# deveshv-99/mlir-HashJoin

Measured on AMD Instinct MI355X. Metric: probed tuples/sec + joined rows/sec, |R|=|S|=2^28 int64 keys, higher is better.
Workload: dtype int64

## Files before the change

### mlir-hashjoin_amd/csrc/hj_capi.cpp

```cpp
#include <hip/hip_runtime.h>

#include <cstdio>
#include <cstdlib>
#include <atomic>
#include <cmath>
#include <cstring>
#include <map>
#include <mutex>
#include <string>
#include <functional>
#include <thread>
#include <type_traits>
#include <vector>

#include "hj.h"
#include "hj_internal.h"

using hj::kNarrow;
using hj::kWide;

namespace {

thread_local std::string g_err;

// ... 384 lines not shown
}

hj::BucketSet bucket_set(SetBufs &sb) {
    hj::BucketSet b;
    b.rows = sb.rows.p;
    b.bbin = (unsigned *)sb.bbin.p;
    b.bfill = (unsigned *)sb.bfill.p;
    b.runs = (unsigned long long *)sb.runs.p;
    b.rstart = (unsigned long long *)sb.rstart.p;
    b.max_buckets = sb.max_buckets;
    b.max_rows = sb.max_rows;
    b.max_runs = sb.max_runs;
    return b;
}

int ensure_radix_scratch(hj_ctx *c, SetBufs &fin, int64_t n, bool wide, const hj::RadixPlan &pl, int routed_src = 0) {
    const size_t P = size_t(1) << pl.total_bits, esz = wide ? 16 : 8;
    HJ_TRY(ensure_set(fin, hj::radix_need(n, pl, true, routed_src), esz, P, hj::kFinalPbl));
    if (pl.passes > 1) HJ_TRY(ensure_set(c->tset, hj::radix_need(n, pl, false, routed_src), esz, P, hj::kPassPbl));
    HJ_TRY(ensure_buf(c->nb, 16));
    HJ_TRY(ensure_buf(c->pcur, (P + 1) * 8));
    HJ_TRY(ensure_buf(c->rcur, (P + 1) * 8));
    HJ_TRY(ensure_buf(c->tile_start, (P + 1) * 4));
    HJ_TRY(ensure_buf(c->tile_owner, (size_t)hj::radix_tiles(n, (int)P) * 4));
    HJ_TRY(ensure_buf(c->tdesc, (size_t)hj::radix_tiles(n, (int)P) * 16));
    HJ_TRY(ensure_buf(c->wstart, 1025 * 4));
    const size_t items = (size_t)hj::radix_join_items(pl, fin.max_runs);
    HJ_TRY(ensure_buf(c->work_start, (size_t)hj::radix_work_words(pl, fin.max_runs) * 4));
    HJ_TRY(ensure_buf(c->work_desc, items * hj::radix_item_desc_bytes()));
    HJ_TRY(ensure_buf(c->scan_sums, ((P + 1) / 8192 + 2) * 8));
    HJ_TRY(ensure_buf(c->raw_cnt, 2 * hj::kRawCntWords * 8));
    {
        const size_t had = c->scan_state.bytes;
        HJ_TRY(ensure_buf(c->scan_state, ((P + 1) / 1024 + 4) * 8));
        if (c->scan_state.bytes != had) HJ_HIP(hipMemset(c->scan_state.p, 0, c->scan_state.bytes));
    }
    return HJ_OK;
}

hj::RadixWork radix_work(hj_ctx *c) {
    hj::RadixWork w;
    w.tmp = bucket_set(c->tset);
    w.nb = (unsigned *)c->nb.p;
    w.pcur = (unsigned long long *)c->pcur.p;
    w.rcur = (unsigned long long *)c->rcur.p;
    w.tile_start = (unsigned *)c->tile_start.p;
    w.tile_owner = (unsigned *)c->tile_owner.p;
    w.tdesc = c->tdesc.p;
    w.wstart = (unsigned *)c->wstart.p;
    w.scan_sums = (unsigned long long *)c->scan_sums.p;
    w.scan_state = (unsigned long long *)c->scan_state.p;
    w.raw_cnt = (unsigned long long *)c->raw_cnt.p;
    w.work_start = (unsigned *)c->work_start.p;
    w.work_desc = c->work_desc.p;
    return w;
}

int choose_strategy(const hj_ctx *c, int64_t n_build) {
    if (c->strategy == HJ_STRATEGY_GLOBAL || c->strategy == HJ_STRATEGY_RADIX) return c->strategy;
    if (n_build >= kRadixMinRows) return HJ_STRATEGY_RADIX;
    if (n_build >= kDualMinBuildRows && c->probe_hint >= radix_probe_min_rows(n_build)) return HJ_STRATEGY_RADIX;
    return HJ_STRATEGY_GLOBAL;
}

struct RadixSrc {
    hj::SrcDev src;
    const uint64_t *counts = nullptr;
// ... 1837 lines not shown
```

### mlir-hashjoin_amd/csrc/hj_radix.hip

```cpp
#include <cstdint>
#include <cstdlib>
#include <type_traits>

#include "hj.h"
#include "hj_internal.h"

namespace hj {
namespace {

typedef unsigned long long u64;
constexpr int kTile = 4096;
constexpr int kPassThreads = 1024;
constexpr int kPassRows = kTile / kPassThreads;
constexpr int kMaxFan = 512;
constexpr int kSmallPassThreads = 512;
constexpr int kSmallFan = 256;
constexpr int kJoinItems = 5;
constexpr int kJoinSub = 8;
constexpr int kPackedRow = 3;
constexpr int kBucketed = 4;
constexpr unsigned kNoBucket = 0xFFFFFFFFu;

__device__ __forceinline__ u64 rhash(u64 k) { return radix_hash(k); }

// ... 111 lines not shown
__global__ __launch_bounds__(1024) void k_scan_blocks(u64 *a, u64 n, u64 *sums) {
    __shared__ u64 wsum[16];
    const u64 base = (u64)blockIdx.x * kScanBlock + (u64)threadIdx.x * kScanPer;
    u64 v[kScanPer], s = 0;
#pragma unroll
    for (int i = 0; i < kScanPer; ++i) {
        v[i] = (base + i < n) ? a[base + i] : 0ull;
        s += v[i];
    }
    u64 total;
    u64 run = block_excl_scan<1024>(s, wsum, &total);
#pragma unroll
    for (int i = 0; i < kScanPer; ++i) {
        if (base + i < n) a[base + i] = run;
        run += v[i];
    }
    if (threadIdx.x == 0) sums[blockIdx.x] = total;
}

__global__ __launch_bounds__(1024) void k_scan_add(u64 *a, u64 n, const u64 *sums) {
    __shared__ u64 wsum[16];
    if (blockIdx.x == 0) return;
    u64 v = 0;
    for (unsigned i = threadIdx.x; i < blockIdx.x; i += 1024) v += sums[i];
    u64 add;
    block_excl_scan<1024>(v, wsum, &add);
    const u64 base = (u64)blockIdx.x * kScanBlock;
    for (int i = threadIdx.x; i < kScanBlock; i += 1024)
        if (base + i < n) a[base + i] += add;
}

__device__ __forceinline__ unsigned runs_of(unsigned fill) { return (fill + (1u << kRunLog) - 1) >> kRunLog; }

constexpr u64 kLbAgg = 1ull << 62, kLbInc = 2ull << 62, kLbVal = (1ull << 62) - 1;
constexpr int kLbThreads = 256, kLbPer = 4, kLbTile = kLbThreads * kLbPer;

struct ChunkMapArgs {
    const u64 *off_a, *off_b;
    unsigned chunk;
    bool split;
    unsigned *start, *owner;
};

template <bool MAP>
__global__ __launch_bounds__(kLbThreads) void k_scan_lb(u64 *a, u64 n, u64 *state, ChunkMapArgs mp) {
    __shared__ u64 wsum[16];
    __shared__ u64 s_pre;
    __shared__ unsigned s_tile;
    const unsigned nt = (unsigned)((n + kLbTile - 1) / kLbTile);
    if (threadIdx.x == 0) s_tile = (unsigned)atomicAdd(&state[nt], 1ull);
    __syncthreads();
    const unsigned t = s_tile;
    const u64 base = (u64)t * kLbTile + (u64)threadIdx.x * kLbPer;
    u64 v[kLbPer], s = 0;
#pragma unroll
    for (int i = 0; i < kLbPer; ++i) {
        const u64 e = base + i;
        if constexpr (MAP) {
            v[i] = 0ull;
            if (e + 1 < n) {
                const u64 len = mp.off_a[e + 1] - mp.off_a[e];
                const bool live = mp.off_b ? (mp.off_b[e + 1] > mp.off_b[e]) : true;
                const u64 c = live ? (len + mp.chunk - 1) / mp.chunk : 0ull;
                v[i] = mp.split && c >= 2 ? c | (c << 31) : c;
            }
        } else {
            v[i] = e < n ? a[e] : 0ull;
        }
        s += v[i];
    }
    u64 total;
    u64 run = block_excl_scan<kLbThreads>(s, wsum, &total);
    if (threadIdx.x < 64) {
        const unsigned lane = threadIdx.x;
        u64 pre = 0;
        if (t == 0) {
            if (lane == 0) atomicExch(&state[0], kLbInc | total);
        } else {
            if (lane == 0) atomicExch(&state[t], kLbAgg | total);
            for (unsigned w = t; w > 0;) {
                const u64 x = lane < w ? atomicOr(&state[w - 1 - lane], 0ull) : kLbInc;
                const u64 inc = __ballot((x >> 62) == 2ull), none = __ballot((x >> 62) == 0ull);
                const u64 upto = inc ? (inc & (~inc + 1ull)) * 2ull - 1ull : ~0ull;
                if (none & upto) {
                    __builtin_amdgcn_s_sleep(1);
                    continue;
                }
                pre += wave_incl_add64((upto >> lane) & 1ull && lane < w ? (x & kLbVal) : 0ull);
                pre = __shfl(pre, 63);
                if (inc) break;
                w = w > 64u ? w - 64u : 0u;
            }
            if (lane == 0) atomicExch(&state[t], kLbInc | (pre + total));
        }
        if (lane == 0) s_pre = pre;
    }
    __syncthreads();
    run += s_pre;
#pragma unroll
    for (int i = 0; i < kLbPer; ++i) {
        const u64 e = base + i;
        if (e < n) {
            if constexpr (MAP) {
                const unsigned lo = (unsigned)(run & 0x7FFFFFFFull);
                a[e] = ((run >> 31) << 32) | lo;
                mp.start[e] = lo;
                const unsigned c = (unsigned)(v[i] & 0x7FFFFFFFull);
                for (unsigned k = 0; k < c; ++k) mp.owner[lo + k] = (unsigned)e;
            } else {
                a[e] = run;
            }
        }
        run += v[i];
    }
    __syncthreads();
    if (threadIdx.x == 0) {
        __threadfence();
        if (atomicAdd(&state[nt + 1], 1ull) == (u64)nt - 1ull) {
            __threadfence();
            for (unsigned k = 0; k < nt + 2; ++k) atomicExch(&state[k], 0ull);
        }
    }
}

struct PassArgs {
    SrcDev in;
    u64 n;
    bool cols_aligned;
    const void *in_rows;
    const u64 *in_runs;
    const u64 *in_rstart;
    u64 in_max_rows, in_max_runs;
    const unsigned *tile_start;
    const struct TileDesc *tdesc;
    int nseg;
    void *out_rows;
    unsigned *bbin, *bfill, *nb;
    const unsigned *wstart;
    unsigned max_buckets;
    int out_pbl;
    int shift;
    int fbits;
    u64 *prof = nullptr;
    u64 *rcnt = nullptr;
    const u64 *slot_base = nullptr;
    u64 out_max_rows = 0;
    int hash_top = 0;
    unsigned tile_rows = kTile;
};

struct TileDesc {
    u64 lo;
    unsigned cnt, seg;
};

// ... 463 lines not shown
        zero_a[i] = 0ull;
        zero_b[i] = 0ull;
    }
    if (blockIdx.x != 0) return;
    const unsigned w = threadIdx.x;
    const unsigned T_ = bucketed ? a.tile_start[a.nseg] : (unsigned)((a.n + a.tile_rows - 1) / a.tile_rows);
    u64 q = 0;
    if (w < G) {
        const unsigned t0 = (unsigned)((u64)w * T_ / G), t1 = (unsigned)((u64)(w + 1) * T_ / G);
        if (t1 > t0) {
            const u64 segs = bucketed ? (u64)(a.tdesc[t1 - 1].seg - a.tdesc[t0].seg + 1) : 1ull;
            const u64 PB = 1ull << a.out_pbl;
            q = ((u64)(t1 - t0) * a.tile_rows + PB - 1) / PB + segs * (1ull << a.fbits) + 1;
        }
    }
    u64 tot;
    const u64 pre = block_excl_scan<1024>(q, wsum, &tot);
    if (w <= G) wstart[w] = (unsigned)(pre < a.max_buckets ? pre : a.max_buckets);
    if (w == G) *a.nb = (unsigned)(tot < a.max_buckets ? tot : a.max_buckets);
}

constexpr int kPlanSegs = 4096;
struct TilePlanArgs {
    PassArgs a;
    const u64 *rstart;
    unsigned G, tb;
    unsigned *tile_start;
    TileDesc *desc;
    unsigned *wstart;
    u64 *zero_a, *zero_b;
    u64 zero_n;
};

__device__ __forceinline__ void tile_plan_body(const TilePlanArgs &p, unsigned bid, unsigned nblk) {
    const PassArgs &a = p.a;
    const u64 *rstart = p.rstart;
    const unsigned G = p.G, tb = p.tb;
    unsigned *tile_start = p.tile_start;
    TileDesc *desc = p.desc;
    unsigned *wstart = p.wstart;
    u64 *zero_a = p.zero_a, *zero_b = p.zero_b;
    const u64 zero_n = p.zero_n;
    __shared__ unsigned ts[kPlanSegs + 1];
    __shared__ u64 wsum[16];
    constexpr int PER = kPlanSegs / 1024;
    const int nseg = a.nseg;
    const unsigned rpt = a.tile_rows >> kRunLog;
    unsigned c[PER], sum = 0;
#pragma unroll
    for (int i = 0; i < PER; ++i) {
        const int sg = threadIdx.x * PER + i;
        c[i] = sg < nseg ? (unsigned)((rstart[sg + 1] - rstart[sg] + rpt - 1) / rpt) : 0u;
        sum += c[i];
    }
    u64 total;
    u64 run = block_excl_scan<1024>(sum, wsum, &total);
#pragma unroll
    for (int i = 0; i < PER; ++i) {
        const int sg = threadIdx.x * PER + i;
        if (sg < nseg) ts[sg] = (unsigned)run;
        run += c[i];
    }
    if (threadIdx.x == 0) ts[nseg] = (unsigned)total;
    __syncthreads();
    const unsigned T = (unsigned)total;
    auto seg_of_tile = [&](unsigned t) -> unsigned {
        unsigned lo = 0, hi = (unsigned)nseg;
        while (hi - lo > 1) {
            const unsigned mid = (lo + hi) >> 1;
            if (ts[mid] <= t) lo = mid;
            else hi = mid;
        }
        return lo;
    };
    for (unsigned t = bid * 1024 + threadIdx.x; t < T && t < tb; t += nblk * 1024) {
        const unsigned sg = seg_of_tile(t);
        const u64 lo = rstart[sg] + (u64)(t - ts[sg]) * rpt;
        const u64 e = rstart[sg + 1];
        TileDesc d;
        d.lo = lo;
        d.cnt = (unsigned)(e - lo < (u64)rpt ? e - lo : (u64)rpt);
        d.seg = sg;
        desc[t] = d;
    }
    for (u64 i = (u64)bid * 1024 + threadIdx.x; i < zero_n; i += (u64)nblk * 1024) {
        zero_a[i] = 0ull;
        zero_b[i] = 0ull;
    }
    if (bid != 0) return;
    for (int sg = threadIdx.x; sg <= nseg; sg += 1024) tile_start[sg] = ts[sg];
    const unsigned w = threadIdx.x;
    u64 q = 0;
    if (w < G) {
        const unsigned t0 = (unsigned)((u64)w * T / G), t1 = (unsigned)((u64)(w + 1) * T / G);
        if (t1 > t0) {
            const u64 segs = (u64)(seg_of_tile(t1 - 1) - seg_of_tile(t0) + 1);
            const u64 PB = 1ull << a.out_pbl;
            q = ((u64)(t1 - t0) * a.tile_rows + PB - 1) / PB + segs * (1ull << a.fbits) + 1;
        }
    }
    u64 tot;
    const u64 pre = block_excl_scan<1024>(q, wsum, &tot);
    if (w <= G) wstart[w] = (unsigned)(pre < a.max_buckets ? pre : a.max_buckets);
    if (w == G) *a.nb = (unsigned)(tot < a.max_buckets ? tot : a.max_buckets);
}

__global__ __launch_bounds__(1024) void k_tile_plan(TilePlanArgs p) { tile_plan_body(p, blockIdx.x, gridDim.x); }

constexpr int kListPer = 4;
constexpr int kListLds = 4096;


struct PlaceArgs {
    const unsigned *bbin, *bfill, *nb;
    unsigned max_buckets;
    int pbl;
    const u64 *rstart;
    u64 *rcur, *runs;
    int P;
    const u64 *raw = nullptr;
};
static_assert(kRawCntWords == (u64)kPlanSegs + 1, "raw count words: a plan's segments + 1");

__device__ __forceinline__ void bplace_body(const PlaceArgs &pa, unsigned bid) {
    const unsigned *bbin = pa.bbin, *bfill = pa.bfill, *nb = pa.nb;
    const unsigned max_buckets = pa.max_buckets;
    const int pbl = pa.pbl;
    const u64 *rstart = pa.rstart;
    u64 *rcur = pa.rcur, *runs = pa.runs;
    const int P = pa.P;
    __shared__ unsigned cr[kListLds];
    __shared__ u64 cbr[kListLds];
    const unsigned n = *nb < max_buckets ? *nb : max_buckets;
    const u64 base = (u64)bid * 1024 * kListPer;
    if (base >= n) return;
    const unsigned lane_ = threadIdx.x & 63u;
    auto put_runs = [&](bool ok, u64 j, unsigned f, u64 at) {
        const int rl = pbl > kRunLog ? (pbl - kRunLog < 6 ? pbl - kRunLog : 6) : 0;
        const unsigned R = 1u << rl, k0 = lane_ & (R - 1u);
        for (unsigned b0 = 0; b0 < 64u; b0 += 64u >> rl) {
            const int src = (int)(b0 + (lane_ >> rl));
            const bool o = __shfl((int)ok, src) != 0;
            const unsigned fs = (unsigned)__shfl((int)f, src);
            const u64 js = ((u64)(unsigned)__shfl((int)(j >> 32), src) << 32) | (unsigned)__shfl((int)j, src);
            const u64 as = ((u64)(unsigned)__shfl((int)(at >> 32), src) << 32) | (unsigned)__shfl((int)at, src);
            for (unsigned k = k0; o && (k << kRunLog) < fs; k += R) {
                const unsigned cnt = fs - (k << kRunLog) < (1u << kRunLog) ? fs - (k << kRunLog) : (1u << kRunLog);
                runs[as + k] = ((((u64)js << pbl) + ((u64)k << kRunLog)) << 7) | cnt;
            }
        }
    };
    if (P > kListLds) {
        const unsigned lane = threadIdx.x & 63u;
        unsigned bi[kListPer], fi[kListPer], pre[kListPer], l0i[kListPer];
        u64 ri[kListPer];
#pragma unroll
        for (int i = 0; i < kListPer; ++i) {
            const u64 j = base + (u64)i * 1024 + threadIdx.x;
            bi[i] = j < n ? bbin[j] : kNoBucket;
            const bool valid = bi[i] < (unsigned)P;
            fi[i] = valid ? bfill[j] : 0u;
            const unsigned nr = runs_of(fi[i]);
            const u64 vm = __ballot(valid);
            l0i[i] = vm ? (unsigned)__ffsll((long long)vm) - 1u : 64u;
            ri[i] = 0ull;
            pre[i] = 0u;
            if (!vm) continue;
            const unsigned b0 = (unsigned)__builtin_amdgcn_readlane((int)bi[i], (int)l0i[i]);
            const bool same = valid && bi[i] == b0;
            const unsigned v = same ? nr : 0u;
            const unsigned incl = wave_incl_add(v);
            const unsigned tot = (unsigned)__builtin_amdgcn_readlane((int)incl, 63);
            pre[i] = same ? incl - v : ~0u;
            if (valid && !same) ri[i] = atomicAdd(&rcur[bi[i]], (u64)nr);
            if (lane == l0i[i]) ri[i] = atomicAdd(&rcur[b0], (u64)tot);
        }
#pragma unroll
        for (int i = 0; i < kListPer; ++i) {
            if (l0i[i] == 64u) continue;
            const unsigned b0 = (unsigned)__builtin_amdgcn_readlane((int)bi[i], (int)l0i[i]);
            const u64 g = ((u64)(unsigned)__builtin_amdgcn_readlane((int)(ri[i] >> 32), (int)l0i[i]) << 32) |
                          (u64)(unsigned)__builtin_amdgcn_readlane((int)ri[i], (int)l0i[i]);
            const bool ok = bi[i] < (unsigned)P;
            const u64 j = base + (u64)i * 1024 + threadIdx.x;
            const u64 at = !ok ? 0ull : (pre[i] != ~0u ? rstart[b0] + g + pre[i] : rstart[bi[i]] + ri[i]);
            put_runs(ok, j, fi[i], at);
        }
        return;
    }
    for (int i = threadIdx.x; i < P; i += 1024) cr[i] = 0u;
    __syncthreads();
    unsigned rr[kListPer], bn[kListPer], fl[kListPer];
#pragma unroll
    for (int i = 0; i < kListPer; ++i) {
        const u64 j = base + (u64)i * 1024 + threadIdx.x;
        bn[i] = j < n ? bbin[j] : kNoBucket;
        if (bn[i] >= (unsigned)P) bn[i] = kNoBucket;
        fl[i] = bn[i] != kNoBucket ? bfill[j] : 0u;
        if (bn[i] != kNoBucket) rr[i] = atomicAdd(&cr[bn[i]], runs_of(fl[i]));
    }
    __syncthreads();
    for (int i = threadIdx.x; i < P; i += 1024)
        if (cr[i]) cbr[i] = rstart[i] + atomicAdd(&rcur[i], (u64)cr[i]);
    __syncthreads();
#pragma unroll
    for (int i = 0; i < kListPer; ++i) {
        const u64 j = base + (u64)i * 1024 + threadIdx.x;
        const bool ok = bn[i] != kNoBucket;
        put_runs(ok, j, fl[i], ok ? cbr[bn[i]] + rr[i] : 0ull);
    }
}

__global__ __launch_bounds__(1024) void k_bplace(PlaceArgs pa) { bplace_body(pa, blockIdx.x); }

__global__ __launch_bounds__(1024) void k_place_plan(PlaceArgs pa, unsigned nplace, TilePlanArgs tp) {
    __shared__ u64 rs[kPlanSegs + 1];
    if (pa.raw) {
        __shared__ u64 wsum[16];
        constexpr int PER = (kPlanSegs + 1 + 1023) / 1024;
        const int n = pa.P + 1;
        u64 v[PER], sum = 0;
#pragma unroll
        for (int i = 0; i < PER; ++i) {
            const int e = threadIdx.x * PER + i;
            v[i] = e < n ? pa.raw[e] : 0ull;
            sum += v[i];
        }
        u64 total;
        u64 run = block_excl_scan<1024>(sum, wsum, &total);
#pragma unroll
        for (int i = 0; i < PER; ++i) {
            const int e = threadIdx.x * PER + i;
            if (e < n) {
                rs[e] = run;
                if (blockIdx.x == 0) ((u64 *)pa.rstart)[e] = run;
            }
            run += v[i];
        }
        __syncthreads();
        pa.rstart = rs;
        tp.rstart = rs;
    }
    if (blockIdx.x < nplace) bplace_body(pa, blockIdx.x);
    else tile_plan_body(tp, blockIdx.x - nplace, gridDim.x - nplace);
}

struct JoinArgs {
    const void *r, *s;
    const u64 *r_runs, *s_runs;
    const u64 *r_rstart, *s_rstart;
    int P;
    const unsigned *work_start;
    const struct ItemDesc *desc;
    int tshift;
    void *out_r, *out_s;
    long long cap;
    u64 *counter;
    u64 *dup_flag;
    unsigned *defer = nullptr, *defer_n = nullptr;
    const unsigned *list = nullptr, *list_n = nullptr;
    const u64 *sample = nullptr;
    unsigned modes = 7u;
    unsigned *next_item = nullptr;
    bool empty_s = false;
    bool all_if_mode2 = false;
    const u64 *skip_if_set = nullptr;
};

constexpr unsigned kModeUnique = 1u, kModeSome = 2u, kModeMostlyRepeated = 4u;
constexpr unsigned kModesAll = kModeUnique | kModeSome | kModeMostlyRepeated;
constexpr int kSampleParts = 64;

typedef __attribute__((address_space(4))) const u64 cu64_t;
__device__ __forceinline__ u64 sload(const u64 *p) { return *(cu64_t *)p; }

__host__ __device__ __forceinline__ int sample_mode(u64 rows, u64 repeats) {
    return repeats * 4 > rows ? 2 : (repeats * 64 >= rows && repeats ? 1 : 0);
// ... 2429 lines not shown
        a.in = src;
        a.n = n;
        a.cols_aligned = ((((uintptr_t)src.key) | ((uintptr_t)src.pay)) & 15) == 0;
        a.in_rows = prev ? prev->rows : nullptr;
        a.in_runs = prev ? prev->runs : nullptr;
        a.in_rstart = prev ? prev->rstart : nullptr;
        a.in_max_rows = prev ? prev->max_rows : 0;
        a.in_max_runs = prev ? prev->max_runs : 0;
        a.tile_start = ws.tile_start;
        a.tdesc = nullptr;
        a.nseg = nseg;
        a.out_rows = dst.rows;
        a.bbin = dst.bbin;
        a.bfill = dst.bfill;
        a.nb = nbw;
        {
            const u64 by_rows = dst.max_rows >> pl.pbl[pass];
            a.max_buckets = (unsigned)(by_rows < dst.max_buckets ? by_rows : dst.max_buckets);
        }
        a.out_pbl = pl.pbl[pass];
        a.shift = shift;
        a.fbits = fb;
        a.tile_rows = pass_tile_rows(fb, wide);
        a.wstart = ws.wstart;
        const u64 P = (u64)nseg << fb;
        const bool fuse = ws.raw_cnt && pass + 1 < pl.passes && P <= (u64)kPlanSegs;
        u64 *cnt = fuse ? ws.raw_cnt + (u64)(pass & 1) * kRawCntWords : dst.rstart;
        a.rcnt = n > 0 ? cnt : nullptr;
        if (grid > 1023) return hipErrorInvalidValue;
        const unsigned zgrid = blocks_for(P + 1, 1024);
        if (prev && nseg <= kPlanSegs) {
            const u64 tb = radix_tiles((long long)n, nseg);
            a.tdesc = (const TileDesc *)ws.tdesc;
            unsigned pg = blocks_for(tb, 1024);
            if (pg < zgrid) pg = zgrid;
            if (pg > 1024) pg = 1024;
            TilePlanArgs tp{a, (const u64 *)prev->rstart, grid, (unsigned)tb, ws.tile_start, (TileDesc *)ws.tdesc,
                            ws.wstart, cnt, rcur, P + 1};
            if (pending) hipLaunchKernelGGL(k_place_plan, dim3(np_prev + pg), dim3(1024), 0, st, pa_prev, np_prev, tp);
            else hipLaunchKernelGGL(k_tile_plan, dim3(pg), dim3(1024), 0, st, tp);
            pending = false;
        } else {
            place_alone();
            if (prev) {
                const unsigned rpt = a.tile_rows >> kRunLog;
                chunk_map(prev->rstart, nullptr, nseg, rpt, ws.tile_start, ws.tile_owner, ws.pcur, ws.scan_sums, st,
                          (u64)n / (u64)(nseg > 0 ? nseg : 1) / (u64)a.tile_rows);
                const u64 tb = radix_tiles((long long)n, nseg);
                hipLaunchKernelGGL(k_tile_desc, dim3(blocks_for(tb, 256)), dim3(256), 0, st,
                                   (const unsigned *)ws.tile_start, (const unsigned *)ws.tile_owner,
                                   (const u64 *)prev->rstart, nseg, (unsigned)tb, (TileDesc *)ws.tdesc, rpt);
                a.tdesc = (const TileDesc *)ws.tdesc;
            }
            hipLaunchKernelGGL(k_id_plan, dim3(zgrid < 1024 ? zgrid : 1024), dim3(1024), 0, st, a, prev != nullptr, grid,
                               ws.wstart, cnt, rcur, P + 1);
        }
        if (n > 0) {
#define HJ_PASS(W, FORM)                                                                                    \
    do {                                                                                                    \
        if (small)                                                                                          \
            hipLaunchKernelGGL((k_pass<W, FORM, 0, false, kSmallPassThreads, kSmallFan,                     \
                                       W ? kPassRows : kSmallNarrowRows>),                                  \
                               dim3(grid), dim3(kSmallPassThreads), 0, st, a);                              \
        else hipLaunchKernelGGL((k_pass<W, FORM>), dim3(grid), dim3(kPassThreads), 0, st, a);               \
    } while (0)
            if (prev) {
                if (wide) HJ_PASS(true, kBucketed);
                else HJ_PASS(false, kBucketed);
            } else if (wide) {
// ... 410 lines not shown
```

### mlir-hashjoin_amd/micro/pass_micro.hip

```cpp
#include "../csrc/hj_radix.hip"

#include <cstdio>
#include <algorithm>
#include <vector>
#ifndef PHASE_ABL
#define PHASE_ABL 8
#endif

#define CK(x) do { hipError_t e = (x); if (e != hipSuccess) { printf("HIP %s at %d\n", hipGetErrorString(e), __LINE__); exit(1);} } while (0)
using namespace hj;
typedef unsigned long long u64;

__global__ void k_fill(ulonglong2 *r, u64 n, int skew) {
    const u64 i = (u64)blockIdx.x * 256 + threadIdx.x;
    if (i >= n) return;
    u64 k = fmix64(i * 7 + 1);
    if (skew) {
        const unsigned j = (unsigned)(fmix64(i ^ 0x5EED) % 1000u);
        if (j < 31) k = j < 16 ? 11ull : (j < 25 ? 22ull : 33ull);
    }
    r[i] = make_ulonglong2(k, i);
}

int main(int argc, char **argv) {
// ... 86 lines not shown
            }
            for (int k = 0; k < 5; ++k) printf("  phase %-38s %10.0f cycles  %5.1f %%\n", names[k], m[k], 100.0 * m[k] / tot);
            a.prof = nullptr;
            CK(hipFree(prof));
        }
    }
    {
        RadixPlan p1{};
        p1.passes = 1;
        p1.bits[0] = 9;
        p1.pbl[0] = kPassPbl;
        p1.total_bits = 9;
        const int P1 = 512;
        RadixNeed nd = radix_need((long long)n, p1, true);
        BucketSet b1;
        CK(hipMalloc(&b1.rows, nd.rows * 16));
        CK(hipMalloc(&b1.bbin, nd.buckets * 4));
        CK(hipMalloc(&b1.bfill, nd.buckets * 4));
        CK(hipMalloc(&b1.rstart, (P1 + 1) * 8));
        b1.max_buckets = (unsigned)nd.buckets;
        b1.max_rows = nd.rows;
        b1.max_runs = (nd.rows >> kRunLog) + nd.buckets;
        CK(hipMalloc(&b1.runs, b1.max_runs * 8));
        const int P2 = P1 << 8;
        RadixWork ws{};
        CK(hipMalloc(&ws.nb, 64));
        CK(hipMalloc(&ws.pcur, (P2 + 1) * 8));
        CK(hipMalloc(&ws.rcur, (P2 + 1) * 8));
        CK(hipMalloc(&ws.tile_start, (P2 + 1) * 4));
        CK(hipMalloc(&ws.tile_owner, radix_tiles((long long)n, P2) * 4));
        CK(hipMalloc(&ws.tdesc, radix_tiles((long long)n, P2) * 16));
        CK(hipMalloc(&ws.wstart, 1025 * 4));
        CK(hipMalloc(&ws.scan_sums, (P2 / 8192 + 2) * 8));
        CK(hipMalloc(&ws.scan_state, (P2 / 1024 + 4) * 8));
        CK(hipMemset(ws.scan_state, 0, (P2 / 1024 + 4) * 8));
        SrcDev src{};
        src.form = kPacked64;
        src.key = in;
        src.n = (long long)n;
        CK(radix_partition(src, true, p1, ws, b1, 0));
        chunk_map(b1.rstart, nullptr, P1, (unsigned)(kTile >> kRunLog), ws.tile_start, ws.tile_owner, ws.pcur,
                  ws.scan_sums, 0);
        {
            const u64 tb = radix_tiles((long long)n, P1);
            hipLaunchKernelGGL(k_tile_desc, dim3(blocks_for(tb, 256)), dim3(256), 0, 0, (const unsigned *)ws.tile_start,
                               (const unsigned *)ws.tile_owner, (const u64 *)b1.rstart, P1, (unsigned)tb,
                               (TileDesc *)ws.tdesc, (unsigned)(kTile >> kRunLog));
        }
        CK(hipDeviceSynchronize());
        unsigned ntiles = 0;
        u64 nruns = 0;
        CK(hipMemcpy(&ntiles, ws.tile_start + P1, 4, hipMemcpyDeviceToHost));
        CK(hipMemcpy(&nruns, b1.rstart + P1, 8, hipMemcpyDeviceToHost));
        printf("pass-1 set: %llu runs (%.3f x n/64), %u pass-2 tiles (%.3f x n/4096)\n", nruns,
               nruns / (double)(n >> 6), ntiles, ntiles / (double)(n >> 12));
        PassArgs b{};
        b.n = n;
        b.in_rows = b1.rows;
        b.in_runs = b1.runs;
        b.in_rstart = b1.rstart;
        b.in_max_rows = b1.max_rows;
        b.in_max_runs = b1.max_runs;
        b.tile_start = ws.tile_start;
        b.tdesc = (const TileDesc *)ws.tdesc;
        b.nseg = P1;
        b.out_rows = out;
        b.bbin = bbin;
        b.bfill = bfill;
// ... 83 lines not shown
```

### mlir-hashjoin_amd/micro/runs_micro.hip

```cpp
#include "../csrc/hj_radix.hip"

#include <cstdio>
#include <vector>

#define CK(x) do { hipError_t e = (x); if (e != hipSuccess) { printf("HIP %s at %d\n", hipGetErrorString(e), __LINE__); exit(1);} } while (0)
using namespace hj;
typedef unsigned long long u64;

__global__ void k_fill64(u64 *k, u64 *p, u64 n) {
    const u64 i = (u64)blockIdx.x * 256 + threadIdx.x;
    if (i < n) { k[i] = fmix64(i * 7 + 1); p[i] = i; }
}
__global__ void k_fill32(int *k, u64 n) {
    const u64 i = (u64)blockIdx.x * 256 + threadIdx.x;
    if (i < n) k[i] = (int)(fmix64(i * 3 + 5) % 1000000000ull) + 1;
}

template <class T> T *dalloc(u64 n) { T *p; CK(hipMalloc(&p, n * sizeof(T) + 64)); return p; }

void run(bool wide, u64 n, int lim_a, int lim_b) {
    const RadixPlan pl = radix_plan((long long)n, 0, wide);
    const int P = 1 << pl.total_bits;
    const size_t esz = wide ? 16 : 8;
    RadixNeed nf = radix_need((long long)n, pl, true), nt = radix_need((long long)n, pl, false);
    auto mkset = [&](RadixNeed nd, int parts) {
        BucketSet b{};
        b.rows = dalloc<char>(nd.rows * esz);
        b.bbin = dalloc<unsigned>(nd.buckets);
        b.bfill = dalloc<unsigned>(nd.buckets);
        b.rstart = dalloc<u64>((u64)parts + 1);
        b.max_buckets = (unsigned)nd.buckets;
        b.max_rows = nd.rows;
        b.max_runs = (nd.rows >> kRunLog) + nd.buckets;
        b.runs = dalloc<u64>(b.max_runs);
        return b;
    };
    BucketSet fin = mkset(nf, P);
    RadixWork ws{};
    ws.tmp = mkset(nt, P);
    ws.nb = dalloc<unsigned>(16);
    ws.pcur = dalloc<u64>(P + 1);
    ws.rcur = dalloc<u64>(P + 1);
    ws.tile_start = dalloc<unsigned>(P + 1);
    ws.tile_owner = dalloc<unsigned>(radix_tiles((long long)n, P));
    ws.tdesc = dalloc<char>(radix_tiles((long long)n, P) * 16);
    ws.wstart = dalloc<unsigned>(1025);
    ws.scan_sums = dalloc<u64>(P / 8192 + 2);
    ws.scan_state = dalloc<u64>(P / 1024 + 4);
    CK(hipMemset(ws.scan_state, 0, (P / 1024 + 4) * 8));
    SrcDev src{};
    src.n = (long long)n;
    if (wide) {
        u64 *k = dalloc<u64>(n), *p = dalloc<u64>(n);
        hipLaunchKernelGGL(k_fill64, dim3((n + 255) / 256), dim3(256), 0, 0, k, p, n);
        src.key = k;
        src.pay = p;
        src.form = kCols64;
    } else {
        int *k = dalloc<int>(n);
        hipLaunchKernelGGL(k_fill32, dim3((n + 255) / 256), dim3(256), 0, 0, k, n);
        src.key = k;
        src.form = kCol32;
    }
    CK(radix_partition(src, wide, pl, ws, fin, 0));
    CK(hipDeviceSynchronize());
    std::vector<u64> rs(P + 1);
    CK(hipMemcpy(rs.data(), fin.rstart, (P + 1) * 8ull, hipMemcpyDeviceToHost));
    std::vector<u64> hist(257, 0);
    u64 over_a = 0, over_b = 0, mx = 0;
    for (int p = 0; p < P; ++p) {
        const u64 r = rs[p + 1] - rs[p];
        hist[r < 256 ? r : 256]++;
        over_a += r > (u64)lim_a;
        over_b += r > (u64)lim_b;
        mx = r > mx ? r : mx;
    }
    printf("%s n=%llu plan %d passes (%d+%d bits), %d partitions, %.1f rows/partition, %llu runs (%.3f x n/64), max %llu\n",
           wide ? "int64" : "i32", n, pl.passes, pl.bits[0], pl.bits[1], P, (double)n / P, rs[P],
           rs[P] / (double)(n >> 6), mx);
    printf("  partitions over %d runs: %.2f %%, over %d runs: %.2f %%\n", lim_a, 100.0 * over_a / P, lim_b,
           100.0 * over_b / P);
    printf("  runs: count\n");
// ... 10 lines not shown
```

### mlir-hashjoin_amd/micro/skew_micro.hip

```cpp
#include "../csrc/hj_radix.hip"

#include <algorithm>
#include <cstdio>
#include <vector>

#define CK(x) do { hipError_t e = (x); if (e != hipSuccess) { printf("HIP %s at %d\n", hipGetErrorString(e), __LINE__); exit(1);} } while (0)
using namespace hj;
typedef unsigned long long u64;

__global__ void k_fill(ulonglong2 *r, u64 n, int skew) {
    const u64 i = (u64)blockIdx.x * 256 + threadIdx.x;
    if (i >= n) return;
    u64 k = fmix64(i * 7 + 1);
    if (skew) {
        const unsigned j = (unsigned)(fmix64(i ^ 0x5EED) % 1000u);
        if (j < 31) k = j < 16 ? 11ull : (j < 25 ? 22ull : 33ull);
    }
    r[i] = make_ulonglong2(k, i);
}

int main() {
    const u64 n = 1ull << 28;
    int cus = 0;
    CK(hipDeviceGetAttribute(&cus, hipDeviceAttributeMultiprocessorCount, 0));
// ... 4 lines not shown
    CK(hipMalloc(&out, maxb * 512 * 16));
    CK(hipMalloc(&bbin, maxb * 4));
    CK(hipMalloc(&bfill, maxb * 4));
    CK(hipMalloc(&nb, 64));
    CK(hipMalloc(&wst, 1025 * 4));
    hipEvent_t e0, e1;
    CK(hipEventCreate(&e0));
    CK(hipEventCreate(&e1));
    RadixPlan p1{};
    p1.passes = 1;
    p1.bits[0] = 9;
    p1.pbl[0] = kPassPbl;
    p1.total_bits = 9;
    const int P1 = 512, P2 = P1 << 8;
    RadixNeed nd = radix_need((long long)n, p1, true);
    BucketSet b1;
    CK(hipMalloc(&b1.rows, nd.rows * 16));
    CK(hipMalloc(&b1.bbin, nd.buckets * 4));
    CK(hipMalloc(&b1.bfill, nd.buckets * 4));
    CK(hipMalloc(&b1.rstart, (P1 + 1) * 8));
    b1.max_buckets = (unsigned)nd.buckets;
    b1.max_rows = nd.rows;
    b1.max_runs = (nd.rows >> kRunLog) + nd.buckets;
    CK(hipMalloc(&b1.runs, (b1.max_runs + kRunPad) * 8));
    RadixWork ws{};
    CK(hipMalloc(&ws.nb, 64));
    CK(hipMalloc(&ws.pcur, (P2 + 1) * 8));
    CK(hipMalloc(&ws.rcur, (P2 + 1) * 8));
    CK(hipMalloc(&ws.tile_start, (P2 + 1) * 4));
    CK(hipMalloc(&ws.tile_owner, radix_tiles((long long)n, P2) * 4));
    CK(hipMalloc(&ws.tdesc, radix_tiles((long long)n, P2) * 16));
    CK(hipMalloc(&ws.wstart, 1025 * 4));
    CK(hipMalloc(&ws.scan_sums, (P2 / 8192 + 2) * 8));
    CK(hipMalloc(&ws.scan_state, (P2 / 1024 + 4) * 8));
    constexpr int NT = kSmallPassThreads, FM = kSmallFan, IT = kPassRows, TR = NT * IT;
    const unsigned grid = 2u * (unsigned)cus;
    u64 *prof;
    CK(hipMalloc(&prof, grid * 8 * sizeof(u64)));
    for (int skew : {0, 1}) {
        hipLaunchKernelGGL(k_fill, dim3(n / 256), dim3(256), 0, 0, in, n, skew);
        CK(hipMemset(ws.scan_state, 0, (P2 / 1024 + 4) * 8));
        SrcDev src{};
        src.form = kPacked64;
        src.key = in;
        src.n = (long long)n;
        CK(radix_partition(src, true, p1, ws, b1, 0));
        chunk_map(b1.rstart, nullptr, P1, (unsigned)(TR >> kRunLog), ws.tile_start, ws.tile_owner, ws.pcur,
                  ws.scan_sums, 0);
        const u64 tb = radix_tiles((long long)n, P1);
        hipLaunchKernelGGL(k_tile_desc, dim3(blocks_for(tb, 256)), dim3(256), 0, 0, (const unsigned *)ws.tile_start,
                           (const unsigned *)ws.tile_owner, (const u64 *)b1.rstart, P1, (unsigned)tb,
                           (TileDesc *)ws.tdesc, (unsigned)(TR >> kRunLog));
        CK(hipDeviceSynchronize());
        unsigned ntiles = 0;
        CK(hipMemcpy(&ntiles, ws.tile_start + P1, 4, hipMemcpyDeviceToHost));
        std::vector<u64> rs(P1 + 1);
        CK(hipMemcpy(rs.data(), b1.rstart, (P1 + 1) * 8, hipMemcpyDeviceToHost));
        u64 mx = 0;
        for (int p = 0; p < P1; ++p) mx = std::max(mx, rs[p + 1] - rs[p]);
        printf("== skew %d: pass-1 segments 512, largest %llu runs (mean %.0f); %u pass-2 tiles of %d rows\n", skew, mx,
               rs[P1] / 512.0, ntiles, TR);
        PassArgs b{};
        b.n = n;
        b.in_rows = b1.rows;
        b.in_runs = b1.runs;
        b.in_rstart = b1.rstart;
        b.in_max_rows = b1.max_rows;
        b.in_max_runs = b1.max_runs;
        b.tile_start = ws.tile_start;
        b.tdesc = (const TileDesc *)ws.tdesc;
        b.nseg = P1;
        b.out_rows = out;
        b.bbin = bbin;
        b.bfill = bfill;
// ... 59 lines not shown
```

Baseline: 32.50 billion.

## Double-buffer decoupled-lookback state, window bucket placement, size plan grid to free CUs

Measured after the change: 32.69 billion, median of 6. Within noise of the previous version (+0.6%).

```diff
diff --git a/mlir-hashjoin_amd/csrc/hj_capi.cpp b/mlir-hashjoin_amd/csrc/hj_capi.cpp
--- a/mlir-hashjoin_amd/csrc/hj_capi.cpp
+++ b/mlir-hashjoin_amd/csrc/hj_capi.cpp
@@ -440,7 +440,7 @@
     HJ_TRY(ensure_buf(c->raw_cnt, 2 * hj::kRawCntWords * 8));
     {
         const size_t had = c->scan_state.bytes;
-        HJ_TRY(ensure_buf(c->scan_state, ((P + 1) / 1024 + 4) * 8));
+        HJ_TRY(ensure_buf(c->scan_state, (2 * ((P + 1) / 1024) + 8) * 8));
         if (c->scan_state.bytes != had) HJ_HIP(hipMemset(c->scan_state.p, 0, c->scan_state.bytes));
     }
     return HJ_OK;
diff --git a/mlir-hashjoin_amd/csrc/hj_radix.hip b/mlir-hashjoin_amd/csrc/hj_radix.hip
--- a/mlir-hashjoin_amd/csrc/hj_radix.hip
+++ b/mlir-hashjoin_amd/csrc/hj_radix.hip
@@ -167,6 +167,20 @@
 
 __device__ __forceinline__ unsigned runs_of(unsigned fill) { return (fill + (1u << kRunLog) - 1) >> kRunLog; }
 
+#ifdef HJ_LIST_PROF
+constexpr unsigned kLprofRows = 4096;
+__device__ u64 d_lprof[kLprofRows][8];
+bool g_lprof_wide_grid = false;
+#define HJ_LPROF(row, s)                                                                                        \
+    do {                                                                                                        \
+        if (threadIdx.x == 0 && (row) < kLprofRows)                                                             \
+            d_lprof[row][s] = (s) == 0 || (s) == 7 ? wall_clock64() : __builtin_amdgcn_s_memtime();             \
+    } while (0)
+#else
+#define HJ_LPROF(row, s) do { } while (0)
+#endif
+
+constexpr u64 kLbTick = (1ull << 24) - 1;
 constexpr u64 kLbAgg = 1ull << 62, kLbInc = 2ull << 62, kLbVal = (1ull << 62) - 1;
 constexpr int kLbThreads = 256, kLbPer = 4, kLbTile = kLbThreads * kLbPer;
 
@@ -181,11 +195,16 @@
 __global__ __launch_bounds__(kLbThreads) void k_scan_lb(u64 *a, u64 n, u64 *state, ChunkMapArgs mp) {
     __shared__ u64 wsum[16];
     __shared__ u64 s_pre;
-    __shared__ unsigned s_tile;
+    __shared__ u64 s_word;
     const unsigned nt = (unsigned)((n + kLbTile - 1) / kLbTile);
-    if (threadIdx.x == 0) s_tile = (unsigned)atomicAdd(&state[nt], 1ull);
+    HJ_LPROF(3072u + blockIdx.x, 0);
+    HJ_LPROF(3072u + blockIdx.x, 1);
+    if (threadIdx.x == 0) s_word = atomicAdd(&state[0], 1ull);
     __syncthreads();
-    const unsigned t = s_tile;
+    const unsigned t = (unsigned)(s_word & kLbTick), left = (unsigned)((s_word >> 24) & kLbTick);
+    const unsigned set = (unsigned)(s_word >> 48) & 1u;
+    u64 *tw = state + 2 + set;
+    HJ_LPROF(3072u + blockIdx.x, 2);
     const u64 base = (u64)t * kLbTile + (u64)threadIdx.x * kLbPer;
     u64 v[kLbPer], s = 0;
 #pragma unroll
@@ -206,15 +225,16 @@
     }
     u64 total;
     u64 run = block_excl_scan<kLbThreads>(s, wsum, &total);
+    HJ_LPROF(3072u + blockIdx.x, 3);
     if (threadIdx.x < 64) {
         const unsigned lane = threadIdx.x;
         u64 pre = 0;
         if (t == 0) {
-            if (lane == 0) atomicExch(&state[0], kLbInc | total);
+            if (lane == 0) atomicExch(&tw[0], kLbInc | total);
         } else {
-            if (lane == 0) atomicExch(&state[t], kLbAgg | total);
+            if (lane == 0) atomicExch(&tw[2u * t], kLbAgg | total);
             for (unsigned w = t; w > 0;) {
-                const u64 x = lane < w ? atomicOr(&state[w - 1 - lane], 0ull) : kLbInc;
+                const u64 x = lane < w ? atomicOr(&tw[2u * (w - 1 - lane)], 0ull) : kLbInc;
                 const u64 inc = __ballot((x >> 62) == 2ull), none = __ballot((x >> 62) == 0ull);
                 const u64 upto = inc ? (inc & (~inc + 1ull)) * 2ull - 1ull : ~0ull;
                 if (none & upto) {
@@ -226,11 +246,12 @@
                 if (inc) break;
                 w = w > 64u ? w - 64u : 0u;
             }
-            if (lane == 0) atomicExch(&state[t], kLbInc | (pre + total));
+            if (lane == 0) atomicExch(&tw[2u * t], kLbInc | (pre + total));
         }
         if (lane == 0) s_pre = pre;
     }
     __syncthreads();
+    HJ_LPROF(3072u + blockIdx.x, 4);
     run += s_pre;
 #pragma unroll
     for (int i = 0; i < kLbPer; ++i) {
@@ -248,14 +269,12 @@
         }
         run += v[i];
     }
-    __syncthreads();
-    if (threadIdx.x == 0) {
-        __threadfence();
-        if (atomicAdd(&state[nt + 1], 1ull) == (u64)nt - 1ull) {
-            __threadfence();
-            for (unsigned k = 0; k < nt + 2; ++k) atomicExch(&state[k], 0ull);
-        }
-    }
+    HJ_LPROF(3072u + blockIdx.x, 5);
+    for (u64 w = (u64)t + (u64)threadIdx.x * nt; w < left; w += (u64)kLbThreads * nt)
+        atomicExch(&state[2 + 2 * w + (set ^ 1u)], 0ull);
+    if (threadIdx.x == 0 && t == nt - 1) atomicExch(&state[0], ((u64)(set ^ 1u) << 48) | ((u64)nt << 24));
+    HJ_LPROF(3072u + blockIdx.x, 6);
+    HJ_LPROF(3072u + blockIdx.x, 7);
 }
 
 struct PassArgs {
@@ -785,7 +804,7 @@
     u64 zero_n;
 };
 
-__device__ __forceinline__ void tile_plan_body(const TilePlanArgs &p, unsigned bid, unsigned nblk) {
+__device__ __forceinline__ void tile_plan_body(const TilePlanArgs &p, unsigned bid, unsigned nblk, unsigned prow) {
     const PassArgs &a = p.a;
     const u64 *rstart = p.rstart;
     const unsigned G = p.G, tb = p.tb;
@@ -816,6 +835,7 @@
     }
     if (threadIdx.x == 0) ts[nseg] = (unsigned)total;
     __syncthreads();
+    HJ_LPROF(prow, 3);
     const unsigned T = (unsigned)total;
     auto seg_of_tile = [&](unsigned t) -> unsigned {
         unsigned lo = 0, hi = (unsigned)nseg;
@@ -836,10 +856,12 @@
         d.seg = sg;
         desc[t] = d;
     }
+    HJ_LPROF(prow, 4);
     for (u64 i = (u64)bid * 1024 + threadIdx.x; i < zero_n; i += (u64)nblk * 1024) {
         zero_a[i] = 0ull;
         zero_b[i] = 0ull;
     }
+    HJ_LPROF(prow, 5);
     if (bid != 0) return;
     for (int sg = threadIdx.x; sg <= nseg; sg += 1024) tile_start[sg] = ts[sg];
     const unsigned w = threadIdx.x;
@@ -856,11 +878,14 @@
     const u64 pre = block_excl_scan<1024>(q, wsum, &tot);
     if (w <= G) wstart[w] = (unsigned)(pre < a.max_buckets ? pre : a.max_buckets);
     if (w == G) *a.nb = (unsigned)(tot < a.max_buckets ? tot : a.max_buckets);
-}
-
-__global__ __launch_bounds__(1024) void k_tile_plan(TilePlanArgs p) { tile_plan_body(p, blockIdx.x, gridDim.x); }
-
-constexpr int kListPer = 4;
+    HJ_LPROF(prow, 6);
+}
+
+__global__ __launch_bounds__(1024) void k_tile_plan(TilePlanArgs p) {
+    tile_plan_body(p, blockIdx.x, gridDim.x, blockIdx.x);
+}
+
+constexpr int kListPer = 2;
 constexpr int kListLds = 4096;
 
 
@@ -875,7 +900,7 @@
 };
 static_assert(kRawCntWords == (u64)kPlanSegs + 1, "raw count words: a plan's segments + 1");
 
-__device__ __forceinline__ void bplace_body(const PlaceArgs &pa, unsigned bid) {
+__device__ __forceinline__ void bplace_body(const PlaceArgs &pa, unsigned bid, unsigned prow) {
     const unsigned *bbin = pa.bbin, *bfill = pa.bfill, *nb = pa.nb;
     const unsigned max_buckets = pa.max_buckets;
     const int pbl = pa.pbl;
@@ -884,6 +909,7 @@
     const int P = pa.P;
     __shared__ unsigned cr[kListLds];
     __shared__ u64 cbr[kListLds];
+    __shared__ unsigned s_wb;
     const unsigned n = *nb < max_buckets ? *nb : max_buckets;
     const u64 base = (u64)bid * 1024 * kListPer;
     if (base >= n) return;
@@ -903,71 +929,83 @@
             }
         }
     };
-    if (P > kListLds) {
-        const unsigned lane = threadIdx.x & 63u;
-        unsigned bi[kListPer], fi[kListPer], pre[kListPer], l0i[kListPer];
-        u64 ri[kListPer];
-#pragma unroll
-        for (int i = 0; i < kListPer; ++i) {
-            const u64 j = base + (u64)i * 1024 + threadIdx.x;
-            bi[i] = j < n ? bbin[j] : kNoBucket;
-            const bool valid = bi[i] < (unsigned)P;
-            fi[i] = valid ? bfill[j] : 0u;
-            const unsigned nr = runs_of(fi[i]);
-            const u64 vm = __ballot(valid);
-            l0i[i] = vm ? (unsigned)__ffsll((long long)vm) - 1u : 64u;
-            ri[i] = 0ull;
-            pre[i] = 0u;
-            if (!vm) continue;
-            const unsigned b0 = (unsigned)__builtin_amdgcn_readlane((int)bi[i], (int)l0i[i]);
-            const bool same = valid && bi[i] == b0;
-            const unsigned v = same ? nr : 0u;
-            const unsigned incl = wave_incl_add(v);
-            const unsigned tot = (unsigned)__builtin_amdgcn_readlane((int)incl, 63);
-            pre[i] = same ? incl - v : ~0u;
-            if (valid && !same) ri[i] = atomicAdd(&rcur[bi[i]], (u64)nr);
-            if (lane == l0i[i]) ri[i] = atomicAdd(&rcur[b0], (u64)tot);
-        }
-#pragma unroll
-        for (int i = 0; i < kListPer; ++i) {
-            if (l0i[i] == 64u) continue;
-            const unsigned b0 = (unsigned)__builtin_amdgcn_readlane((int)bi[i], (int)l0i[i]);
-            const u64 g = ((u64)(unsigned)__builtin_amdgcn_readlane((int)(ri[i] >> 32), (int)l0i[i]) << 32) |
-                          (u64)(unsigned)__builtin_amdgcn_readlane((int)ri[i], (int)l0i[i]);
-            const bool ok = bi[i] < (unsigned)P;
-            const u64 j = base + (u64)i * 1024 + threadIdx.x;
-            const u64 at = !ok ? 0ull : (pre[i] != ~0u ? rstart[b0] + g + pre[i] : rstart[bi[i]] + ri[i]);
-            put_runs(ok, j, fi[i], at);
-        }
-        return;
-    }
-    for (int i = threadIdx.x; i < P; i += 1024) cr[i] = 0u;
-    __syncthreads();
-    unsigned rr[kListPer], bn[kListPer], fl[kListPer];
+    for (int i = threadIdx.x; i < kListLds; i += 1024) cr[i] = 0u;
+    if (threadIdx.x == 0) s_wb = P > kListLds ? kNoBucket : 0u;
+    unsigned bn[kListPer], fl[kListPer], rr[kListPer], lo = kNoBucket;
+    u64 ri[kListPer];
 #pragma unroll
     for (int i = 0; i < kListPer; ++i) {
         const u64 j = base + (u64)i * 1024 + threadIdx.x;
         bn[i] = j < n ? bbin[j] : kNoBucket;
+        const unsigned f = j < n ? bfill[j] : 0u;
         if (bn[i] >= (unsigned)P) bn[i] = kNoBucket;
-        fl[i] = bn[i] != kNoBucket ? bfill[j] : 0u;
-        if (bn[i] != kNoBucket) rr[i] = atomicAdd(&cr[bn[i]], runs_of(fl[i]));
+        fl[i] = bn[i] != kNoBucket ? f : 0u;
+        lo = bn[i] < lo ? bn[i] : lo;
+        rr[i] = 0u;
+        ri[i] = 0ull;
     }
     __syncthreads();
-    for (int i = threadIdx.x; i < P; i += 1024)
-        if (cr[i]) cbr[i] = rstart[i] + atomicAdd(&rcur[i], (u64)cr[i]);
+    if (P > kListLds) {
+#pragma unroll
+        for (int d = 32; d > 0; d >>= 1) {
+            const unsigned o = (unsigned)__shfl_xor((int)lo, d);
+            lo = o < lo ? o : lo;
+        }
+        if (lane_ == 0 && lo != kNoBucket) atomicMin(&s_wb, lo);
+        __syncthreads();
+    }
+    const unsigned wb = s_wb;
+    HJ_LPROF(prow, 3);
+#pragma unroll
+    for (int i = 0; i < kListPer; ++i) {
+        if (bn[i] == kNoBucket) continue;
+        const unsigned w = bn[i] - wb;
+        if (w < (unsigned)kListLds) rr[i] = atomicAdd(&cr[w], runs_of(fl[i]));
+        else ri[i] = atomicAdd(&rcur[bn[i]], (u64)runs_of(fl[i]));
+    }
     __syncthreads();
+    {
+        constexpr int CP = kListLds / 1024;
+        unsigned c[CP];
+        u64 g[CP];
+#pragma unroll
+        for (int k = 0; k < CP; ++k) {
+            const unsigned w = threadIdx.x + k * 1024;
+            c[k] = cr[w];
+            g[k] = 0ull;
+            if (c[k]) g[k] = atomicAdd(&rcur[wb + w], (u64)c[k]);
+        }
+#pragma unroll
+        for (int k = 0; k < CP; ++k) {
+            const unsigned w = threadIdx.x + k * 1024;
+            if (c[k]) cbr[w] = rstart[wb + w] + g[k];
+        }
+    }
+    __syncthreads();
+    HJ_LPROF(prow, 4);
 #pragma unroll
     for (int i = 0; i < kListPer; ++i) {
         const u64 j = base + (u64)i * 1024 + threadIdx.x;
         const bool ok = bn[i] != kNoBucket;
-        put_runs(ok, j, fl[i], ok ? cbr[bn[i]] + rr[i] : 0ull);
-    }
-}
-
-__global__ __launch_bounds__(1024) void k_bplace(PlaceArgs pa) { bplace_body(pa, blockIdx.x); }
+        const unsigned w = bn[i] - wb;
+        const u64 at = !ok ? 0ull : (w < (unsigned)kListLds ? cbr[w] + rr[i] : rstart[bn[i]] + ri[i]);
+        put_runs(ok, j, fl[i], at);
+    }
+    HJ_LPROF(prow, 5);
+}
+
+__global__ __launch_bounds__(1024) void k_bplace(PlaceArgs pa) {
+    HJ_LPROF(2048u + blockIdx.x, 0);
+    HJ_LPROF(2048u + blockIdx.x, 1);
+    HJ_LPROF(2048u + blockIdx.x, 2);
+    bplace_body(pa, blockIdx.x, 2048u + blockIdx.x);
+    HJ_LPROF(2048u + blockIdx.x, 7);
+}
 
 __global__ __launch_bounds__(1024) void k_place_plan(PlaceArgs pa, unsigned nplace, TilePlanArgs tp) {
     __shared__ u64 rs[kPlanSegs + 1];
+    HJ_LPROF(blockIdx.x, 0);
+    HJ_LPROF(blockIdx.x, 1);
     if (pa.raw) {
         __shared__ u64 wsum[16];
         constexpr int PER = (kPlanSegs + 1 + 1023) / 1024;
@@ -994,8 +1032,10 @@
         pa.rstart = rs;
         tp.rstart = rs;
     }
-    if (blockIdx.x < nplace) bplace_body(pa, blockIdx.x);
-    else tile_plan_body(tp, blockIdx.x - nplace, gridDim.x - nplace);
+    HJ_LPROF(blockIdx.x, 2);
+    if (blockIdx.x < nplace) bplace_body(pa, blockIdx.x, blockIdx.x);
+    else tile_plan_body(tp, blockIdx.x - nplace, gridDim.x - nplace, blockIdx.x);
+    HJ_LPROF(blockIdx.x, 7);
 }
 
 struct JoinArgs {
@@ -3491,9 +3531,21 @@
         if (prev && nseg <= kPlanSegs) {
             const u64 tb = radix_tiles((long long)n, nseg);
             a.tdesc = (const TileDesc *)ws.tdesc;
-            unsigned pg = blocks_for(tb, 1024);
+            const u64 rpt = a.tile_rows >> kRunLog;
+            u64 tmax = prev->max_runs / rpt + (u64)nseg + 1;
+            if (tmax > tb) tmax = tb;
+            unsigned pg = blocks_for(tmax, 1024);
             if (pg < zgrid) pg = zgrid;
-            if (pg > 1024) pg = 1024;
+            const unsigned np = pending ? np_prev : 0u, cus = (unsigned)cu_count();
+            const unsigned room = cus > np + 32u ? cus - np : 32u;
+            if (pg > room) pg = room;
+#ifdef HJ_LIST_PROF
+            if (g_lprof_wide_grid) {
+                pg = blocks_for(tb, 1024);
+                if (pg < zgrid) pg = zgrid;
+                if (pg > 1024) pg = 1024;
+            }
+#endif
             TilePlanArgs tp{a, (const u64 *)prev->rstart, grid, (unsigned)tb, ws.tile_start, (TileDesc *)ws.tdesc,
                             ws.wstart, cnt, rcur, P + 1};
             if (pending) hipLaunchKernelGGL(k_place_plan, dim3(np_prev + pg), dim3(1024), 0, st, pa_prev, np_prev, tp);
diff --git a/mlir-hashjoin_amd/micro/list_micro.hip b/mlir-hashjoin_amd/micro/list_micro.hip
--- /dev/null
+++ b/mlir-hashjoin_amd/micro/list_micro.hip
@@ -0,0 +1,140 @@
+#ifndef HJ_LIST_PROF
+#define HJ_LIST_PROF
+#endif
+#include "../csrc/hj_radix.hip"
+
+#include <algorithm>
+#include <cstdio>
+#include <vector>
+
+#define CK(x) do { hipError_t e = (x); if (e != hipSuccess) { printf("HIP %s at %d\n", hipGetErrorString(e), __LINE__); exit(1);} } while (0)
+using namespace hj;
+typedef unsigned long long u64;
+
+__global__ void k_fill(ulonglong2 *r, u64 n) {
+    const u64 i = (u64)blockIdx.x * 256 + threadIdx.x;
+    if (i < n) r[i] = make_ulonglong2(fmix64(i * 7 + 1), i);
+}
+
+static void alloc_set(BucketSet &b, const RadixNeed &nd, u64 P) {
+    CK(hipMalloc(&b.rows, nd.rows * 16));
+    CK(hipMalloc(&b.bbin, nd.buckets * 4));
+    CK(hipMalloc(&b.bfill, nd.buckets * 4));
+    CK(hipMalloc(&b.rstart, (P + 1) * 8));
+    b.max_buckets = (unsigned)nd.buckets;
+    b.max_rows = nd.rows;
+    b.max_runs = (nd.rows >> kRunLog) + nd.buckets;
+    CK(hipMalloc(&b.runs, (b.max_runs + kRunPad) * 8));
+}
+
+static void report(const char *name, const std::vector<u64> &h, unsigned r0, unsigned r1, int last,
+                   const char *const *phase) {
+    u64 t0 = ~0ull;
+    for (unsigned r = 0; r < kLprofRows; ++r)
+        if (h[r * 8] && h[r * 8] < t0) t0 = h[r * 8];
+    unsigned nblk = 0;
+    double st_sum = 0, st_max = 0, en_sum = 0, en_max = 0, ph_sum[8] = {0}, ph_max[8] = {0};
+    double ticks = 0, wall = 0;
+    for (unsigned r = r0; r < r1 && r < kLprofRows; ++r) {
+        const u64 *m = &h[r * 8];
+        if (!m[0] || !m[7] || !m[last]) continue;
+        ++nblk;
+        const double st = (m[0] - t0) * 0.01, en = (m[7] - t0) * 0.01;
+        st_sum += st, en_sum += en;
+        st_max = std::max(st_max, st), en_max = std::max(en_max, en);
+        ticks += (double)(m[last] - m[1]), wall += (double)(m[7] - m[0]) * 0.01;
+    }
+    if (!nblk) {
+        printf("  %-28s no blocks\n", name);
+        return;
+    }
+    const double us_per_tick = ticks > 0 ? wall / ticks : 0;
+    for (unsigned r = r0; r < r1 && r < kLprofRows; ++r) {
+        const u64 *m = &h[r * 8];
+        if (!m[0] || !m[7] || !m[last]) continue;
+        for (int k = 2; k <= last; ++k) {
+            const double d = (double)(m[k] - m[k - 1]) * us_per_tick;
+            ph_sum[k] += d;
+            ph_max[k] = std::max(ph_max[k], d);
+        }
+    }
+    printf("  %-28s %4u blocks  start mean %6.2f max %6.2f us   end mean %6.2f max %6.2f us\n", name, nblk,
+           st_sum / nblk, st_max, en_sum / nblk, en_max);
+    for (int k = 2; k <= last; ++k)
+        printf("      %-36s mean %6.2f max %6.2f us\n", phase[k], ph_sum[k] / nblk, ph_max[k]);
+}
+
+int main(int argc, char **argv) {
+    const int lg = argc > 1 ? atoi(argv[1]) : 28;
+    const u64 n = 1ull << lg;
+    const RadixPlan pl = radix_plan((long long)n, 0, true);
+    const u64 P = 1ull << pl.total_bits;
+    printf("n = 2^%d, %d passes, bits %d + %d, P = %llu\n", lg, pl.passes, pl.bits[0], pl.bits[1], P);
+    if (pl.passes != 2) {
+        printf("this micro reads a 2-pass plan\n");
+        return 1;
+    }
+    ulonglong2 *in;
+    CK(hipMalloc(&in, n * 16));
+    hipLaunchKernelGGL(k_fill, dim3((unsigned)((n + 255) / 256)), dim3(256), 0, 0, in, n);
+    BucketSet out{};
+    RadixWork ws{};
+    alloc_set(out, radix_need((long long)n, pl, true), P);
+    alloc_set(ws.tmp, radix_need((long long)n, pl, false), P);
+    const u64 tiles = radix_tiles((long long)n, (int)P);
+    CK(hipMalloc(&ws.nb, 64));
+    CK(hipMalloc(&ws.pcur, (P + 1) * 8));
+    CK(hipMalloc(&ws.rcur, (P + 1) * 8));
+    CK(hipMalloc(&ws.tile_start, (P + 1) * 4));
+    CK(hipMalloc(&ws.tile_owner, tiles * 4));
+    CK(hipMalloc(&ws.tdesc, tiles * 16));
+    CK(hipMalloc(&ws.wstart, 1025 * 4));
+    CK(hipMalloc(&ws.scan_sums, ((P + 1) / 8192 + 2) * 8));
+    CK(hipMalloc(&ws.scan_state, (2 * ((P + 1) / 1024) + 8) * 8));
+    CK(hipMemset(ws.scan_state, 0, (2 * ((P + 1) / 1024) + 8) * 8));
+    CK(hipMalloc(&ws.raw_cnt, 2 * kRawCntWords * 8));
+    SrcDev src{};
+    src.form = kPacked64;
+    src.key = in;
+    src.n = (long long)n;
+    CK(hipDeviceSynchronize());
+    const unsigned np1 = blocks_for(ws.tmp.max_buckets, 1024 * kListPer);
+    static const char *const place_ph[8] = {"", "", "raw counts scanned", "ids loaded, window known",
+                                            "counted, cursor adds done", "runs written", "", ""};
+    static const char *const plan_ph[8] = {"", "", "raw counts scanned", "tile counts scanned", "descriptors written",
+                                           "counters zeroed", "block 0: id ranges", ""};
+    static const char *const scan_ph[8] = {"", "", "ticket drawn", "loaded and block-scanned", "looked back",
+                                           "stores issued", "other set's words zeroed", ""};
+    for (int wide = 0; wide < 2; ++wide) {
+        g_lprof_wide_grid = wide != 0;
+        CK(radix_partition(src, true, pl, ws, out, 0));
+        CK(hipDeviceSynchronize());
+        void *marks = nullptr;
+        CK(hipGetSymbolAddress(&marks, HIP_SYMBOL(d_lprof)));
+        CK(hipMemset(marks, 0, sizeof(d_lprof)));
+        CK(radix_partition(src, true, pl, ws, out, 0));
+        CK(hipDeviceSynchronize());
+        std::vector<u64> h((size_t)kLprofRows * 8);
+        CK(hipMemcpyFromSymbol(h.data(), HIP_SYMBOL(d_lprof), sizeof(d_lprof)));
+        u64 runs1 = 0, runs2 = 0;
+        unsigned nb[2] = {0, 0};
+        CK(hipMemcpy(&runs1, ws.tmp.rstart + (1u << pl.bits[0]), 8, hipMemcpyDeviceToHost));
+        CK(hipMemcpy(&runs2, out.rstart + P, 8, hipMemcpyDeviceToHost));
+        CK(hipMemcpy(nb, ws.nb, 8, hipMemcpyDeviceToHost));
+        printf("%s plan grid: pass 1 lists %llu runs of %u bucket ids, pass 2 %llu runs of %u ids\n",
+               wide ? "previous (by the descriptor bound)" : "product", runs1, nb[0], runs2, nb[1]);
+        std::vector<u64> a(h), b(h), c(h);
+        for (unsigned r = 0; r < kLprofRows; ++r)
+            for (int k = 0; k < 8; ++k) {
+                if (r >= 2048) a[r * 8 + k] = 0;
+                if (r < 2048 || r >= 3072) b[r * 8 + k] = 0;
+                if (r < 3072) c[r * 8 + k] = 0;
+            }
+        report("k_place_plan place blocks", a, 0, np1, 5, place_ph);
+        report("k_place_plan plan block 0", a, np1, np1 + 1, 6, plan_ph);
+        report("k_place_plan plan blocks", a, np1 + 1, 2048, 5, plan_ph);
+        report("k_scan_lb tiles", c, 3072, 4096, 6, scan_ph);
+        report("k_bplace blocks", b, 2048, 3072, 5, place_ph);
+    }
+    return 0;
+}
diff --git a/mlir-hashjoin_amd/micro/pass_micro.hip b/mlir-hashjoin_amd/micro/pass_micro.hip
--- a/mlir-hashjoin_amd/micro/pass_micro.hip
+++ b/mlir-hashjoin_amd/micro/pass_micro.hip
@@ -142,8 +142,8 @@
         CK(hipMalloc(&ws.tdesc, radix_tiles((long long)n, P2) * 16));
         CK(hipMalloc(&ws.wstart, 1025 * 4));
         CK(hipMalloc(&ws.scan_sums, (P2 / 8192 + 2) * 8));
-        CK(hipMalloc(&ws.scan_state, (P2 / 1024 + 4) * 8));
-        CK(hipMemset(ws.scan_state, 0, (P2 / 1024 + 4) * 8));
+        CK(hipMalloc(&ws.scan_state, (2 * (P2 / 1024) + 8) * 8));
+        CK(hipMemset(ws.scan_state, 0, (2 * (P2 / 1024) + 8) * 8));
         SrcDev src{};
         src.form = kPacked64;
         src.key = in;
diff --git a/mlir-hashjoin_amd/micro/runs_micro.hip b/mlir-hashjoin_amd/micro/runs_micro.hip
--- a/mlir-hashjoin_amd/micro/runs_micro.hip
+++ b/mlir-hashjoin_amd/micro/runs_micro.hip
@@ -46,8 +46,8 @@
     ws.tdesc = dalloc<char>(radix_tiles((long long)n, P) * 16);
     ws.wstart = dalloc<unsigned>(1025);
     ws.scan_sums = dalloc<u64>(P / 8192 + 2);
-    ws.scan_state = dalloc<u64>(P / 1024 + 4);
-    CK(hipMemset(ws.scan_state, 0, (P / 1024 + 4) * 8));
+    ws.scan_state = dalloc<u64>(2 * (P / 1024) + 8);
+    CK(hipMemset(ws.scan_state, 0, (2 * (P / 1024) + 8) * 8));
     SrcDev src{};
     src.n = (long long)n;
     if (wide) {
diff --git a/mlir-hashjoin_amd/micro/skew_micro.hip b/mlir-hashjoin_amd/micro/skew_micro.hip
--- a/mlir-hashjoin_amd/micro/skew_micro.hip
+++ b/mlir-hashjoin_amd/micro/skew_micro.hip
@@ -60,14 +60,14 @@
     CK(hipMalloc(&ws.tdesc, radix_tiles((long long)n, P2) * 16));
     CK(hipMalloc(&ws.wstart, 1025 * 4));
     CK(hipMalloc(&ws.scan_sums, (P2 / 8192 + 2) * 8));
-    CK(hipMalloc(&ws.scan_state, (P2 / 1024 + 4) * 8));
+    CK(hipMalloc(&ws.scan_state, (2 * (P2 / 1024) + 8) * 8));
     constexpr int NT = kSmallPassThreads, FM = kSmallFan, IT = kPassRows, TR = NT * IT;
     const unsigned grid = 2u * (unsigned)cus;
     u64 *prof;
     CK(hipMalloc(&prof, grid * 8 * sizeof(u64)));
     for (int skew : {0, 1}) {
         hipLaunchKernelGGL(k_fill, dim3(n / 256), dim3(256), 0, 0, in, n, skew);
-        CK(hipMemset(ws.scan_state, 0, (P2 / 1024 + 4) * 8));
+        CK(hipMemset(ws.scan_state, 0, (2 * (P2 / 1024) + 8) * 8));
         SrcDev src{};
         src.form = kPacked64;
         src.key = in;
```
